# YuhuaXu/ImageMosaicing

Measured on AMD Instinct MI355X. Metric: image-pairs/sec (detect+match+H+warp), 4000x3000 UAV frames, higher is better.
Workload: dtype i16 fixed-point pyramid filtered in f32 (as the reference's OpenCV), f32 (RANSAC / warp coordinates), int8 MFMA with int32 accumulation (descriptor distances, exact), u8 (pixels); 1 GPU; C3: ONE 500-frame 4000x3000 UAV survey, pair window 2 (499 pairs), SIFT(2000,3,0.01,20) + exact BF match + 3x3 grid select + Ransac2D + MosaicImagesRefined warp; frames=500, pairs=499, frames_per_gpu=500, pairs_per_gpu=499

## Files before the change

imagemosaicing_amd/csrc/sift.hip:

```cpp
#include "common.h"
#include <memory>
#include "detmath.h"
#include <cmath>
#include <type_traits>

namespace {

constexpr int N_LAYERS = 3, N_LEVELS = 6, IMG_BORDER = 5, MAX_INTERP = 5, ORI_BINS = 36, MAX_OCT = 16;
constexpr int FIXPT_SCALE = 48;
constexpr float DOG_THRESHOLD_P1 = 21.0f;
constexpr float HIST_Q = 1024.0f;
constexpr int MAX_R = 16;
constexpr int SIFT_BATCH_MAX = MI355_SIFT_BATCH_MAX;
typedef int16_t lvl_t;

__host__ __device__ __forceinline__ int reflect101(int p, int n) {
    if (n == 1) return 0;
    while (p < 0 || p >= n) { if (p < 0) p = -p; else p = 2 * n - 2 - p; }
    return p;
}

typedef float v2f __attribute__((ext_vector_type(2)));
struct __attribute__((aligned(4))) uint2_a4 { unsigned x, y; };
typedef float v4f __attribute__((ext_vector_type(4)));
// ... 546 lines not shown
        for (int idx = lane; idx < nq; idx += 64) {
            const unsigned g = base + (unsigned)idx;
            if (g >= cap) { *overflow = 1; continue; }
            cand[(size_t)reg * cap + g] = s_rec[wave][idx];
        }
        wave_sync();
        nq = 0;
    };
    auto emit = [&](unsigned hit, int rc, auto in_loop) -> bool {
        constexpr bool IN_LOOP = decltype(in_loop)::value;
        const int nq0 = nq;
        while (__builtin_amdgcn_ballot_w64(hit != 0)) {
            const bool mine = hit != 0;
            const int bb = mine ? __builtin_ctz(hit) : 0;
            hit &= hit - 1;
            const unsigned long long m = __builtin_amdgcn_ballot_w64(mine);
            const int add = __builtin_popcountll(m);
            if (nq + add > XCAP) {
                if constexpr (IN_LOOP) { nq = nq0; return false; }
                else flush();
            }
            if (mine) {
                const int layer = bb / 4 + 1, c = xm + (bb & 3);
                s_rec[wave][nq + __builtin_popcountll(m & ((1ull << lane) - 1ull))] =
                    ((unsigned long long)octave << 48) | ((unsigned long long)layer << 40) | ((unsigned long long)rc << 20) | (unsigned long long)c;
            }
            nq += add;
        }
        return true;
    };
    XH win[3];
    XCen cen[3];
    XRow nxt[XD];
    {
        XRow q; XDog dq;
        load_row(y0 - 1, q); to_dog(q, dq); xrow_extremes(dq, win[0], cen[0]);
        load_row(y0, q); to_dog(q, dq); xrow_extremes(dq, win[1], cen[1]);
#pragma unroll
        for (int d = 0; d < XD; d++) load_row(y0 + 1 + d, nxt[d]);
    }
    int tb = 0, t_slow = -1;
    for (bool done = false; !done;) {
        for (;;) {
            if (tb >= lact) { done = true; break; }
            if (nq > XCAP / 2) break;
            auto step = [&](auto jc) -> bool {
                constexpr int j = decltype(jc)::value;
                const int tt = tb + j;
                if (tt >= lact) return false;
                const int rc = y0 + tt;
                XH& A = win[j % 3]; XH& B = win[(j + 1) % 3]; XH& Cc = win[(j + 2) % 3];
                { XDog dq; to_dog(nxt[j % XD], dq); xrow_extremes(dq, Cc, cen[(j + 2) % 3]); }
                load_row(rc + 1 + XD, nxt[j % XD]);
                const unsigned hit = xtest_rows(A, B, Cc, cen[(j + 1) % 3], xm, clo, chi, rc >= IMG_BORDER && rc < oc.h - IMG_BORDER);
                if (!emit(hit, rc, std::true_type{})) { t_slow = tt; return false; }
                return true;
            };
            if (!static_rows<0, 3 * XD>(step)) { done = true; break; }
            tb += 3 * XD;
        }
        flush();
    }
    if (t_slow >= 0) {
        for (int tt = t_slow; tt < lact; tt++) {
            const int rc = y0 + tt;
            XRow q; XDog A, B, Cc;
            load_row(rc - 1, q); to_dog(q, A);
            load_row(rc, q); to_dog(q, B);
            load_row(rc + 1, q); to_dog(q, Cc);
            emit(xtest_row(A, B, Cc, xm, clo, chi, rc >= IMG_BORDER && rc < oc.h - IMG_BORDER), rc, std::false_type{});
        }
        flush();
    }
}

__global__ __launch_bounds__(256) void refine_kernel(PyrDev P, const unsigned long long* cand_all, const unsigned* cand_counts, unsigned cand_cap, unsigned* cand_total,
                                                     float contrast_thr, float edge_thr, float sigma,
                                                     Refined* out, unsigned* out_count, unsigned out_cap, unsigned* out_resp, BatchStride bs,
                                                     const float* cube_all, unsigned cube_cap) {
    const size_t fr = blockIdx.z, foff = fr * bs.pyr;
    cube_all += fr * bs.cube;
    cand_all += fr * bs.cand; cand_counts += fr * CCNT_STRIDE; cand_total += fr * CNT_STRIDE;
    out += fr * bs.refined; out_count += fr * CNT_STRIDE; out_resp += fr * bs.refined;
    const unsigned reg = blockIdx.y;
    unsigned n = cand_counts[reg * REG_STRIDE];
    if (n > cand_cap) n = cand_cap;
    const unsigned long long* cand = cand_all + (size_t)reg * cand_cap;
    if (blockIdx.x == 0 && blockIdx.y == 0 && threadIdx.x < 64) {
        unsigned tot = cand_counts[threadIdx.x * REG_STRIDE];
        for (int off = 32; off > 0; off >>= 1) tot += __shfl_xor(tot, off);
        if (threadIdx.x == 0) cand_total[0] = tot;
    }
    for (unsigned i = blockIdx.x * blockDim.x + threadIdx.x; i < n; i += gridDim.x * blockDim.x) {
        const unsigned long long pk = cand[i];
        const int o = (int)((pk >> 48) & 0xff);
        int L = (int)((pk >> 40) & 0xff), R = (int)((pk >> 20) & 0xfffff), C = (int)(pk & 0xfffff);
        const unsigned start = ((unsigned)L << 28) | ((unsigned)R << 14) | (unsigned)C;
        const OctaveDev& oc = P.oc[o];
        auto dv = [&](int l, int r, int c) { return dogv(oc, foff, l, r, c); };
        FitOff f = {0.0f, 0.0f, 0.0f};
        int it = 0;
        bool alive = true, accepted = false;
        float contr = 0.0f;
        const bool from_cube = (pk >> 63) != 0;
        const bool can_gather = (oc.w & 1) == 0 && (foff & 1) == 0;
        float cv[27];
        auto gather = [&](int l, int r, int c) {
            const int a0 = (c - 1) & ~1, sh = ((c - 1) & 1) * 16;
            int v[4][9];
#pragma unroll
            for (int q = 0; q < 4; q++) {
                const lvl_t* lp = oc.lv[l - 1 + q] + foff;
#pragma unroll
                for (int dr = 0; dr < 3; dr++) {
                    const uint2_a4 wv = *reinterpret_cast<const uint2_a4*>(lp + (size_t)(r - 1 + dr) * oc.w + a0);
                    const unsigned long long ww = (((unsigned long long)wv.y << 32) | wv.x) >> sh;
                    v[q][dr * 3 + 0] = (int)(short)(ww & 0xffffu); v[q][dr * 3 + 1] = (int)(short)((ww >> 16) & 0xffffu); v[q][dr * 3 + 2] = (int)(short)((ww >> 32) & 0xffffu);
                }
            }
#pragma unroll
            for (int dl = 0; dl < 3; dl++)
#pragma unroll
                for (int e = 0; e < 9; e++) cv[dl * 9 + e] = (float)(v[dl + 1][e] - v[dl][e]);
        };
        if (from_cube || can_gather) {
            for (; it < MAX_INTERP; it++) {
                if (it == 0 && from_cube) {
                    const float* cb = cube_all + (size_t)reg * 32 * cube_cap + i;
#pragma unroll
                    for (int e = 0; e < 27; e++) cv[e] = cb[(size_t)e * cube_cap];
                } else if (can_gather) gather(L, R, C);
                else break;
                const int L0 = L, R0 = R, C0 = C;
                auto dvc = [&](int l, int r, int c) { return cv[(l - L0 + 1) * 9 + (r - R0 + 1) * 3 + (c - C0 + 1)]; };
                f = fit_step(dvc, L, R, C);
                const int stt = fit_state(f);
                if (stt == 1) { alive = false; break; }
                if (stt == 0) { accepted = fit_accept(dvc, L, R, C, f, contrast_thr, edge_thr, contr); alive = accepted; break; }
                C += (int)rintf(f.xc); R += (int)rintf(f.xr); L += (int)rintf(f.xi);
                if (L < 1 || L > N_LAYERS || C < IMG_BORDER || C >= oc.w - IMG_BORDER || R < IMG_BORDER || R >= oc.h - IMG_BORDER) { alive = false; break; }
            }
            if (!alive || (can_gather && !accepted)) continue;
        }
        if (!accepted) {
            for (; it < MAX_INTERP; it++) {
                f = fit_step(dv, L, R, C);
                const int stt = fit_state(f);
                if (stt == 0) break;
                if (stt == 1) { alive = false; break; }
                C += (int)rintf(f.xc); R += (int)rintf(f.xr); L += (int)rintf(f.xi);
                if (L < 1 || L > N_LAYERS || C < IMG_BORDER || C >= oc.w - IMG_BORDER || R < IMG_BORDER || R >= oc.h - IMG_BORDER) { alive = false; break; }
            }
            if (!alive || it >= MAX_INTERP) continue;
            if (!fit_accept(dv, L, R, C, f, contrast_thr, edge_thr, contr)) continue;
        }
        const size_t bit = ((size_t)R * oc.w + C) * 4 + (size_t)L;
        const unsigned mask = 1u << (bit & 31);
        if (!P.mins[o]) {
            const unsigned old = atomicOr(&P.claimed[o][fr * bs.claimed + (bit >> 5)], mask);
            if (old & mask) continue;
        }
        const unsigned long long act = __ballot(1);
        const int leader = __builtin_ctzll(act), lane_id = (int)(threadIdx.x & 63);
        unsigned slot = 0;
        if (lane_id == leader) slot = atomicAdd(out_count, (unsigned)__builtin_popcountll(act));
        slot = __shfl(slot, leader) + (unsigned)__builtin_popcountll(act & ((1ull << lane_id) - 1ull));
        if (slot < out_cap) {
            Refined rr;
            rr.o = o; rr.layer = L; rr.r = R; rr.c = C; rr.xi = f.xi; rr.xr = f.xr; rr.xc = f.xc; rr.contr = contr;
            rr.scl = sigma * det_exp2f(((float)L + f.xi) / (float)N_LAYERS);
            rr.start = start;
            out[slot] = rr;
            out_resp[slot] = __float_as_uint(fabsf(contr));
            if (P.mins[o]) atomicMin(&P.mins[o][fr * bs.mins + bit], start);
        } else if (!P.mins[o]) atomicAnd(&P.claimed[o][fr * bs.claimed + (bit >> 5)], ~mask);
    }
}

__device__ __forceinline__ void unclaim_body(const PyrDev& P, const Refined* ref, const unsigned* ref_count, unsigned ref_cap, const BatchStride& bs, size_t fr, unsigned first, unsigned step) {
    ref += fr * bs.refined; ref_count += fr * CNT_STRIDE;
    unsigned n = *ref_count;
    if (n > ref_cap) n = ref_cap;
    for (unsigned i = first; i < n; i += step) {
        const Refined rr = ref[i];
        const size_t bit = ((size_t)rr.r * P.oc[rr.o].w + rr.c) * 4 + (size_t)rr.layer;
        atomicAnd(&P.claimed[rr.o][fr * bs.claimed + (bit >> 5)], ~(1u << (bit & 31)));
    }
}

__global__ __launch_bounds__(256) void keepall_live_kernel(PyrDev P, const Refined* ref, const unsigned* ref_count, unsigned ref_cap, unsigned* ctrl, unsigned* list, BatchStride bs) {
    const size_t fr = blockIdx.y;
    ref += fr * bs.refined; ref_count += fr * CNT_STRIDE; ctrl += fr * CNT_STRIDE; list += fr * bs.refined;
    unsigned n = *ref_count;
    if (n > ref_cap) n = ref_cap;
    const int lane = threadIdx.x & 63;
    for (unsigned i0 = blockIdx.x * blockDim.x; i0 < n; i0 += gridDim.x * blockDim.x) {
        const unsigned i = i0 + threadIdx.x;
        bool take = false;
        if (i < n) {
            const Refined rr = ref[i];
            const size_t bit = ((size_t)rr.r * P.oc[rr.o].w + rr.c) * 4 + (size_t)rr.layer;
            take = P.mins[rr.o][fr * bs.mins + bit] == rr.start;
        }
        const unsigned long long m = __builtin_amdgcn_ballot_w64(take);
        if (m) {
            const int first = __builtin_ctzll(m);
            unsigned base = 0;
            if (lane == first) base = atomicAdd(&ctrl[2], (unsigned)__builtin_popcountll(m));
            base = __shfl(base, first);
            if (take) list[base + (unsigned)__builtin_popcountll(m & ((1ull << lane) - 1ull))] = i;
        }
    }
}
__global__ __launch_bounds__(256) void keepall_reset_kernel(PyrDev P, const Refined* ref, const unsigned* ref_count, unsigned ref_cap, BatchStride bs) {
    const size_t fr = blockIdx.y;
    ref += fr * bs.refined; ref_count += fr * CNT_STRIDE;
    unsigned n = *ref_count;
    if (n > ref_cap) n = ref_cap;
    for (unsigned i = blockIdx.x * blockDim.x + threadIdx.x; i < n; i += gridDim.x * blockDim.x) {
        const Refined rr = ref[i];
        P.mins[rr.o][fr * bs.mins + ((size_t)rr.r * P.oc[rr.o].w + rr.c) * 4 + (size_t)rr.layer] = 0xffffffffu;
    }
}

struct KpRec {
    unsigned resp_bits; int o, layer, r, c, bin;
    float ptx, pty, scl, angle, xi;
    unsigned start;
};

constexpr int UNCLAIM_WGS = 32;
__global__ __launch_bounds__(1024) void select_unclaim_kernel(PyrDev P, const Refined* ref, BatchStride bs,
                                                              const unsigned* resp , const unsigned* ref_count, unsigned ref_cap,
                                                              unsigned want, unsigned* ctrl , size_t resp_stride,
                                                              unsigned* list ) {
    if (blockIdx.x > 0) { unclaim_body(P, ref, ref_count, ref_cap, bs, blockIdx.y, (blockIdx.x - 1) * 1024 + threadIdx.x, (gridDim.x - 1) * 1024); return; }
    resp += (size_t)blockIdx.y * resp_stride; ref_count += (size_t)blockIdx.y * CNT_STRIDE; ctrl += (size_t)blockIdx.y * CNT_STRIDE;
    list += (size_t)blockIdx.y * resp_stride;
    __shared__ unsigned s_h[16][256];
    __shared__ unsigned s_sel[2], s_cnt;
    const int tid = threadIdx.x, wv = tid >> 6;
    unsigned n = *ref_count;
    if (n > ref_cap) n = ref_cap;
    if (n <= want) {
        if (tid == 0) { ctrl[0] = 0; ctrl[1] = 0; ctrl[2] = n; }
        for (unsigned i = tid; i < n; i += 1024) list[i] = i;
        return;
    }
    const unsigned nr = (n + 1023u) & ~1023u;
    unsigned above = 0, hi_sel = 0;
    for (int pass = 0; pass < 2; pass++) {
        for (int i = tid; i < 16 * 256; i += 1024) (&s_h[0][0])[i] = 0;
        __syncthreads();
        for (unsigned i0 = tid; i0 < nr; i0 += 8 * 1024) {
            unsigned vv[8];
#pragma unroll
            for (int u = 0; u < 8; u++) { const unsigned i = i0 + 1024u * u; vv[u] = i < n ? resp[i] : 0u; }
#pragma unroll
            for (int u = 0; u < 8; u++) {
                if (i0 + 1024u * u >= n) continue;
                const unsigned key = (vv[u] >> 15) & 0xffffu;
                if (pass == 0) atomicAdd(&s_h[wv][key >> 8], 1u);
                else if ((key >> 8) == hi_sel) atomicAdd(&s_h[wv][key & 255u], 1u);
            }
        }
        __syncthreads();
        if (tid < 256) { unsigned t = 0; for (int w = 0; w < 16; w++) t += s_h[w][tid]; s_h[0][tid] = t; }
        __syncthreads();
        if (tid == 0) {
            unsigned cum = above; int b = 255;
            for (; b >= 0; b--) { if (cum + s_h[0][b] >= want) break; cum += s_h[0][b]; }
            if (b < 0) b = 0;
            s_sel[0] = (unsigned)b; s_sel[1] = cum;
        }
        __syncthreads();
        if (pass == 0) { hi_sel = s_sel[0]; above = s_sel[1]; }
        else if (tid == 0) { ctrl[0] = ((hi_sel << 8) | s_sel[0]) << 15; ctrl[1] = 0; s_cnt = 0; }
        __syncthreads();
    }
    const unsigned T = ((hi_sel << 8) | s_sel[0]) << 15;
    const int lane = tid & 63;
    for (unsigned i0 = tid; i0 < nr; i0 += 8 * 1024) {
        unsigned vv[8];
#pragma unroll
        for (int u = 0; u < 8; u++) { const unsigned i = i0 + 1024u * u; vv[u] = i < n ? resp[i] : 0u; }
#pragma unroll
        for (int u = 0; u < 8; u++) {
            const unsigned i = i0 + 1024u * u;
            const bool take = i < n && vv[u] >= T;
            const unsigned long long m = __builtin_amdgcn_ballot_w64(take);
            if (m) {
                const int first = __builtin_ctzll(m);
                unsigned base = 0;
                if (lane == first) base = atomicAdd(&s_cnt, (unsigned)__builtin_popcountll(m));
                base = __shfl(base, first);
                if (take) list[base + (unsigned)__builtin_popcountll(m & ((1ull << lane) - 1ull))] = i;
            }
        }
    }
    __syncthreads();
    if (tid == 0) ctrl[2] = s_cnt;
}

constexpr int OCAP = 256;
__global__ __launch_bounds__(256) void orient_kernel(PyrDev P, const Refined* ref, const unsigned* ref_count, unsigned ref_cap,
                                                     KpRec* out, unsigned* out_resp, unsigned* out_count, unsigned out_cap,
                                                     const unsigned* ctrl, int pass, BatchStride bs, const unsigned* list) {
    const size_t fr = blockIdx.y, foff = fr * bs.pyr;
    ref += fr * bs.refined; ref_count += fr * CNT_STRIDE; out += fr * bs.kps; out_resp += fr * bs.kps; out_count += fr * CNT_STRIDE; ctrl += fr * CNT_STRIDE;
    list += fr * bs.refined;
    __shared__ unsigned long long s_hq[4][ORI_BINS];
    const unsigned Tbits = ctrl[0];
    if (pass == 1 && (ctrl[1] == 0 || Tbits == 0)) return;
    __shared__ float s_hist[4][ORI_BINS + 4];
    __shared__ KpRec s_out[OCAP];
    __shared__ unsigned s_on, s_obase;
    const int tid = threadIdx.x, lane = tid & 63, wv = tid >> 6;
    unsigned n = *ref_count;
    if (n > ref_cap) n = ref_cap;
    if (pass == 0) n = ctrl[2] < n ? ctrl[2] : n;
    if (tid == 0) s_on = 0;
    __syncthreads();
    for (unsigned base = blockIdx.x * 4; base < n; base += gridDim.x * 4) {
        unsigned k = base + wv;
        bool take = false;
        if (k < n) {
            if (pass == 0) { k = list[k]; take = true; }
            else take = __float_as_uint(fabsf(ref[k].contr)) < Tbits;
        }
        if (take) {
            const Refined rr = ref[k];
            const OctaveDev& oc = P.oc[rr.o];
            const lvl_t* img = oc.lv[rr.layer] + foff;
            const int radius = (int)rintf(4.5f * rr.scl);
            const float osig = 1.5f * rr.scl;
            const float expf_scale = -1.0f / (2.0f * osig * osig);
            const int side = 2 * radius + 1, S = side * side;
            if (lane < ORI_BINS) s_hq[wv][lane] = 0ull;
            __builtin_amdgcn_fence(__ATOMIC_ACQ_REL, "workgroup");
            __builtin_amdgcn_wave_barrier();
            const int per = (S + 63) / 64;
            int sc = lane * per, ic = sc / side, jc = sc - ic * side;
            for (int k0 = 0; k0 < per; k0 += 4) {
                float dxv[4], dyv[4]; int d2v[4]; bool okv[4];
#pragma unroll
                for (int u = 0; u < 4; u++) {
                    const int s = k0 + u < per ? sc : S;
                    const int i = ic - radius, j = jc - radius;
                    sc++; jc++;
                    if (jc == side) { jc = 0; ic++; }
                    const int y = rr.r + i, x = rr.c + j;
                    okv[u] = (s < S) && !(y <= 0 || y >= oc.h - 1 || x <= 0 || x >= oc.w - 1);
                    d2v[u] = i * i + j * j;
                    dxv[u] = 0.0f; dyv[u] = 0.0f;
                    if (okv[u]) {
                        dxv[u] = (float)((int)img[(size_t)y * oc.w + x + 1] - (int)img[(size_t)y * oc.w + x - 1]);
                        dyv[u] = (float)((int)img[(size_t)(y - 1) * oc.w + x] - (int)img[(size_t)(y + 1) * oc.w + x]);
                    }
                }
#pragma unroll
                for (int u = 0; u < 4; u++) {
                    if (!okv[u]) continue;
                    const float dx = dxv[u], dy = dyv[u];
                    const float wgt = det_expf((float)d2v[u] * expf_scale);
                    const float ang = det_atan2deg(dy, dx);
                    const float mag = sqrtf(dx * dx + dy * dy);
                    int b = (int)rintf(((float)ORI_BINS / 360.0f) * ang);
                    if (b >= ORI_BINS) b -= ORI_BINS;
                    if (b < 0) b += ORI_BINS;
                    const float t = wgt * mag;
                    atomicAdd(&s_hq[wv][b], (unsigned long long)(long long)(int)rintf(t * HIST_Q));
                }
            }
            __builtin_amdgcn_fence(__ATOMIC_ACQ_REL, "workgroup");
            __builtin_amdgcn_wave_barrier();
            if (lane < ORI_BINS) s_hist[wv][lane] = (float)(long long)s_hq[wv][lane] * (1.0f / HIST_Q);
            __builtin_amdgcn_fence(__ATOMIC_ACQ_REL, "workgroup");
            __builtin_amdgcn_wave_barrier();
            float hs = 0.0f;
            if (lane < ORI_BINS) {
                const float m2 = s_hist[wv][(lane + ORI_BINS - 2) % ORI_BINS], m1 = s_hist[wv][(lane + ORI_BINS - 1) % ORI_BINS];
                const float p1 = s_hist[wv][(lane + 1) % ORI_BINS], p2 = s_hist[wv][(lane + 2) % ORI_BINS];
                hs = ((m2 + p2) * (1.0f / 16.0f) + (m1 + p1) * (4.0f / 16.0f)) + s_hist[wv][lane] * (6.0f / 16.0f);
            }
            float omax = hs;
            for (int off = 32; off > 0; off >>= 1) { const float o2 = __shfl_xor(omax, off); omax = o2 > omax ? o2 : omax; }
            const float hl = __shfl(hs, lane > 0 ? lane - 1 : ORI_BINS - 1);
            const float hr = __shfl(hs, lane < ORI_BINS - 1 ? lane + 1 : 0);
            const float mag_thr = omax * 0.8f;
            if (lane < ORI_BINS && hs > hl && hs > hr && hs >= mag_thr) {
                float bf = (float)lane + (0.5f * (hl - hr)) / ((hl - 2.0f * hs) + hr);
                bf = bf < 0.0f ? (float)ORI_BINS + bf : (bf >= (float)ORI_BINS ? bf - (float)ORI_BINS : bf);
                KpRec kr;
                kr.resp_bits = __float_as_uint(fabsf(rr.contr));
                kr.o = rr.o; kr.layer = rr.layer; kr.r = rr.r; kr.c = rr.c; kr.bin = lane;
                kr.ptx = (float)rr.c + rr.xc; kr.pty = (float)rr.r + rr.xr; kr.scl = rr.scl; kr.xi = rr.xi; kr.start = rr.start;
                kr.angle = (360.0f / (float)ORI_BINS) * bf;
                const unsigned slot = atomicAdd(&s_on, 1u);
                if (slot < OCAP) s_out[slot] = kr;
            }
        }
        __syncthreads();
        const bool last = base + gridDim.x * 4 >= n;
        if (s_on > OCAP - 72 || last) {
            const unsigned cntl = s_on < OCAP ? s_on : OCAP;
            if (tid == 0 && cntl) s_obase = atomicAdd(out_count, cntl);
            __syncthreads();
            for (unsigned i = tid; i < cntl; i += 256) {
                const unsigned g = s_obase + i;
                if (g < out_cap) { out[g] = s_out[i]; out_resp[g] = s_out[i].resp_bits; }
            }
            __syncthreads();
            if (tid == 0) s_on = 0;
            __syncthreads();
        }
    }
}

constexpr int TOPK_CAP = 4096;

struct SelRec { float ptx, pty, scl, angle; int o, layer; };

__device__ __forceinline__ unsigned long long tie_key(const KpRec& k) {
    return ((unsigned long long)k.o << 52) | ((unsigned long long)k.layer << 48) | ((unsigned long long)k.r << 28) | ((unsigned long long)k.c << 8) | (unsigned long long)k.bin;
}

__global__ __launch_bounds__(1024) void topk_kernel(const KpRec* kps, const unsigned* resp, const unsigned* kp_count, unsigned kp_cap, int nfeatures,
                                                    FrameOuts outs, SelRec* out_sel, int* out_n, int* overflow, unsigned* ctrl, int pass, BatchStride bs) {
    const size_t fr = blockIdx.x;
    kps += fr * bs.kps; resp += fr * bs.kps; kp_count += fr * CNT_STRIDE; out_sel += fr * bs.sel; out_n += fr * CNT_STRIDE; overflow += fr * CNT_STRIDE; ctrl += fr * CNT_STRIDE;
    mi355_keypoint* out_kp = outs.kp[0];
#pragma unroll
    for (int q = 1; q < SIFT_BATCH_MAX; q++) if ((int)fr == q) out_kp = outs.kp[q];
    __shared__ unsigned s_hist[256];
    if (pass == 1 && (ctrl[1] == 0 || ctrl[0] == 0)) return;
    __shared__ unsigned s_misc[8];
    __shared__ unsigned long long s_k0[TOPK_CAP];
    __shared__ unsigned long long s_k1[TOPK_CAP];
    __shared__ unsigned s_idx[TOPK_CAP];
    const int tid = threadIdx.x, lane = tid & 63;
    unsigned N = *kp_count;
    if (N > kp_cap) { N = kp_cap; if (tid == 0) *overflow = 1; }
    const unsigned K = (unsigned)nfeatures;
    unsigned thresh = 0;
    if (N > K) {
        unsigned prefix = 0, want = K;
        const unsigned Nr = (N + 1023u) & ~1023u;
        for (int pass = 0; pass < 4; pass++) {
            const int shift = 24 - 8 * pass;
            for (int i = tid; i < 256; i += 1024) s_hist[i] = 0;
            __syncthreads();
            const unsigned himask = pass == 0 ? 0u : (0xffffffffu << (shift + 8));
            for (unsigned i0 = tid; i0 < Nr; i0 += 8 * 1024) {
                unsigned vv[8];
#pragma unroll
                for (int u = 0; u < 8; u++) { const unsigned i = i0 + 1024u * u; vv[u] = i < N ? resp[i] : 0u; }
#pragma unroll
                for (int u = 0; u < 8; u++) {
                    const unsigned i = i0 + 1024u * u;
                    if (i0 + 1024u * u - tid >= Nr) break;
                    const unsigned v = vv[u];
                    const bool valid = (i < N) && ((v & himask) == prefix);
                    const unsigned d = (v >> shift) & 255u;
                    unsigned long long peers = __ballot(valid);
#pragma unroll
                    for (int b = 0; b < 8; b++) {
                        const unsigned long long m = __ballot(valid && ((d >> b) & 1u));
                        peers &= ((d >> b) & 1u) ? m : ~m;
                    }
                    if (valid && (peers & ((1ull << lane) - 1ull)) == 0ull) atomicAdd(&s_hist[d], (unsigned)__popcll(peers));
                }
            }
            __syncthreads();
            if (tid == 0) {
                unsigned cum = 0; int b = 255;
                for (; b >= 0; b--) { if (cum + s_hist[b] >= want) break; cum += s_hist[b]; }
                if (b < 0) b = 0;
                s_misc[0] = (unsigned)b; s_misc[1] = want - cum;
            }
            __syncthreads();
            prefix |= s_misc[0] << shift; want = s_misc[1];
            __syncthreads();
        }
        thresh = prefix;
    }
    if (tid == 0) s_misc[2] = 0;
    for (int i = tid; i < TOPK_CAP; i += 1024) { s_k0[i] = ~0ull; s_k1[i] = ~0ull; s_idx[i] = 0xffffffffu; }
    __syncthreads();
    for (unsigned i0 = tid; i0 < N; i0 += 8 * 1024) {
        unsigned vv[8];
#pragma unroll
        for (int u = 0; u < 8; u++) { const unsigned i = i0 + 1024u * u; vv[u] = i < N ? resp[i] : 0u; }
#pragma unroll
        for (int u = 0; u < 8; u++) {
            const unsigned i = i0 + 1024u * u;
            if (i < N && vv[u] >= thresh) {
                const KpRec k = kps[i];
                const unsigned slot = atomicAdd(&s_misc[2], 1u);
                if (slot < TOPK_CAP) { s_k0[slot] = (unsigned long long)(~k.resp_bits); s_k1[slot] = tie_key(k); s_idx[slot] = i; }
            }
        }
    }
    __syncthreads();
    unsigned M = s_misc[2];
    if (M > TOPK_CAP) { M = TOPK_CAP; if (tid == 0) *overflow = 1; }
    if (N > K && M > (unsigned)SEL_STRIDE && tid == 0) *overflow = 1;
    int SN = 64;
    while ((unsigned)SN < M) SN <<= 1;
    for (int k = 2; k <= SN; k <<= 1) {
        for (int j = k >> 1; j > 0; j >>= 1) {
            for (int i = tid; i < SN; i += 1024) {
                const int ixj = i ^ j;
                if (ixj > i) {
                    const unsigned long long a0 = s_k0[i], a1 = s_k1[i], b0 = s_k0[ixj], b1 = s_k1[ixj];
                    const bool gt = (a0 > b0) || (a0 == b0 && a1 > b1);
                    const bool up = (i & k) == 0;
                    if (gt == up) {
                        s_k0[i] = b0; s_k1[i] = b1; s_k0[ixj] = a0; s_k1[ixj] = a1;
                        const unsigned t = s_idx[i]; s_idx[i] = s_idx[ixj]; s_idx[ixj] = t;
                    }
                }
            }
            __syncthreads();
        }
    }
    const unsigned keep = N > K ? (M < (unsigned)SEL_STRIDE ? M : (unsigned)SEL_STRIDE) : M;
    for (unsigned i = tid; i < keep; i += 1024) {
        const KpRec k = kps[s_idx[i]];
        const float s2 = (float)(1 << k.o);
        mi355_keypoint kp;
        kp.x = k.ptx * s2; kp.y = k.pty * s2; kp.size = (k.scl * s2) * 2.0f; kp.angle = k.angle;
        kp.response = __uint_as_float(k.resp_bits);
        kp.octave = (k.o & 255) | (k.layer << 8) | (((int)rintf((k.xi + 0.5f) * 255.0f)) << 16);
        kp.class_id = -1;
        out_kp[i] = kp;
        SelRec sr; sr.ptx = k.ptx; sr.pty = k.pty; sr.scl = k.scl; sr.angle = k.angle; sr.o = k.o; sr.layer = k.layer;
        out_sel[i] = sr;
    }
    if (tid == 0) {
        *out_n = (int)keep;
        if (pass == 0 && ctrl[0] != 0 && keep < K) ctrl[1] = 1;
    }
}

__global__ __launch_bounds__(256) void keepall_output_kernel(const KpRec* kps, const unsigned* kp_count, unsigned kp_cap, FrameOuts outs, SelRec* out_sel, int* out_n, int* overflow, BatchStride bs) {
    const size_t fr = blockIdx.y;
    kps += fr * bs.kps; kp_count += fr * CNT_STRIDE; out_sel += fr * bs.sel; out_n += fr * CNT_STRIDE; overflow += fr * CNT_STRIDE;
    mi355_keypoint* out_kp = outs.kp[0];
#pragma unroll
    for (int q = 1; q < SIFT_BATCH_MAX; q++) if ((int)fr == q) out_kp = outs.kp[q];
    unsigned N = *kp_count;
    if (N > kp_cap || N > (unsigned)KEEPALL_MAX) {
        if (blockIdx.x == 0 && threadIdx.x == 0) { *overflow = 1; *out_n = 0; }
        return;
    }
    if (blockIdx.x == 0 && threadIdx.x == 0) *out_n = (int)N;
    auto key_of = [](const KpRec& k) { return ((unsigned long long)k.o << 40) | ((unsigned long long)k.start << 6) | (unsigned long long)k.bin; };
    __shared__ unsigned long long s_key[1024];
    const unsigned i = blockIdx.x * 256 + threadIdx.x;
    if (blockIdx.x * 256 >= N) return;
    KpRec mine;
    unsigned long long mk = ~0ull;
    if (i < N) { mine = kps[i]; mk = key_of(mine); }
    unsigned rank = 0;
    for (unsigned t0 = 0; t0 < N; t0 += 1024) {
        __syncthreads();
        for (unsigned q = threadIdx.x; q < 1024; q += 256) s_key[q] = t0 + q < N ? key_of(kps[t0 + q]) : ~0ull;
        __syncthreads();
        const unsigned cntq = N - t0 < 1024 ? N - t0 : 1024;
        for (unsigned q = 0; q < cntq; q++) rank += s_key[q] < mk ? 1u : 0u;
    }
    if (i >= N) return;
    const KpRec& k = mine;
    const float s2 = (float)(1 << k.o);
    mi355_keypoint kp;
    kp.x = k.ptx * s2; kp.y = k.pty * s2; kp.size = (k.scl * s2) * 2.0f; kp.angle = k.angle;
    kp.response = __uint_as_float(k.resp_bits);
    kp.octave = (k.o & 255) | (k.layer << 8) | (((int)rintf((k.xi + 0.5f) * 255.0f)) << 16);
    kp.class_id = -1;
    out_kp[rank] = kp;
    SelRec sr; sr.ptx = k.ptx; sr.pty = k.pty; sr.scl = k.scl; sr.angle = k.angle; sr.o = k.o; sr.layer = k.layer;
    out_sel[rank] = sr;
}

__global__ __launch_bounds__(256) void describe_kernel(PyrDev P, const SelRec* sel, const int* n_sel, FrameOuts outs, BatchStride bs) {
    const size_t fr = blockIdx.y, foff = fr * bs.pyr;
    sel += fr * bs.sel; n_sel += fr * CNT_STRIDE;
    uint8_t* desc = outs.d8[0];
#pragma unroll
    for (int q = 1; q < SIFT_BATCH_MAX; q++) if ((int)fr == q) desc = outs.d8[q];
    constexpr int d = 4, n = 8, HB = (d + 2) * (d + 2) * (n + 2);
    __shared__ unsigned long long s_hq4[4][HB];
    __shared__ float s_dst4[4][128];
    const int lane = threadIdx.x & 63, wv = threadIdx.x >> 6;
    const int kidx = blockIdx.x * 4 + wv;
    if (kidx >= *n_sel) return;
    unsigned long long* s_hq = s_hq4[wv];
    float* s_dst = s_dst4[wv];
    auto wave_sync = [&]() { __builtin_amdgcn_fence(__ATOMIC_ACQ_REL, "workgroup"); __builtin_amdgcn_wave_barrier(); };
    const SelRec k = sel[kidx];
    const OctaveDev& oc = P.oc[k.o];
    const lvl_t* img = oc.lv[k.layer] + foff;
    const int rows = oc.h, cols = oc.w;
    for (int i = lane; i < HB; i += 64) s_hq[i] = 0ull;
    wave_sync();
    const int px = (int)rintf(k.ptx), py = (int)rintf(k.pty);
    float sin_t, cos_t;
    det_sincosdeg(k.angle, sin_t, cos_t);
    const float bins_per_deg = (float)n / 360.0f;
    const float exp_scale = -1.0f / ((float)(d * d) * 0.5f);
    const float hist_width = 3.0f * k.scl;
    const int radius = (int)rintf(hist_width * 1.4142135623730951f * (float)(d + 1) * 0.5f);
    cos_t = cos_t / hist_width; sin_t = sin_t / hist_width;
    const int side = 2 * radius + 1, S = side * side;
    __shared__ int s_q4[4][64 * 5];
    int* s_q = s_q4[wv];
    int qn = 0;
    auto heavy = [&](int packed) {
        const int i = (int)((unsigned)packed >> 16) - 32768, j = (int)((unsigned)packed & 0xffffu) - 32768;
        const float c_rot = (float)j * cos_t - (float)i * sin_t;
        const float r_rot = (float)j * sin_t + (float)i * cos_t;
        float rbin = r_rot + (float)(d / 2) - 0.5f;
        float cbin = c_rot + (float)(d / 2) - 0.5f;
        const int r = py + i, c = px + j;
        const float dx = (float)((int)img[(size_t)r * cols + c + 1] - (int)img[(size_t)r * cols + c - 1]);
        const float dy = (float)((int)img[(size_t)(r - 1) * cols + c] - (int)img[(size_t)(r + 1) * cols + c]);
        const float ori = det_atan2deg(dy, dx);
        const float mag = sqrtf(dx * dx + dy * dy) * det_expf((c_rot * c_rot + r_rot * r_rot) * exp_scale);
        float obin = (ori - k.angle) * bins_per_deg;
        const float r0f = floorf(rbin), c0f = floorf(cbin), o0f = floorf(obin);
        rbin -= r0f; cbin -= c0f; obin -= o0f;
        const int r0 = (int)r0f, c0 = (int)c0f;
        int o0 = (int)o0f;
        if (o0 < 0) o0 += n;
        if (o0 >= n) o0 -= n;
        const float v_r1 = mag * rbin, v_r0 = mag - v_r1;
        const float v_rc11 = v_r1 * cbin, v_rc10 = v_r1 - v_rc11;
        const float v_rc01 = v_r0 * cbin, v_rc00 = v_r0 - v_rc01;
        const float v_rco111 = v_rc11 * obin, v_rco110 = v_rc11 - v_rco111;
        const float v_rco101 = v_rc10 * obin, v_rco100 = v_rc10 - v_rco101;
        const float v_rco011 = v_rc01 * obin, v_rco010 = v_rc01 - v_rco011;
        const float v_rco001 = v_rc00 * obin, v_rco000 = v_rc00 - v_rco001;
        const int idx = ((r0 + 1) * (d + 2) + c0 + 1) * (n + 2) + o0;
#define FIXQ(v) ((unsigned long long)(long long)(int)rintf((v) * HIST_Q))
        atomicAdd(&s_hq[idx], FIXQ(v_rco000)); atomicAdd(&s_hq[idx + 1], FIXQ(v_rco001));
        atomicAdd(&s_hq[idx + (n + 2)], FIXQ(v_rco010)); atomicAdd(&s_hq[idx + (n + 3)], FIXQ(v_rco011));
        atomicAdd(&s_hq[idx + (d + 2) * (n + 2)], FIXQ(v_rco100)); atomicAdd(&s_hq[idx + (d + 2) * (n + 2) + 1], FIXQ(v_rco101));
        atomicAdd(&s_hq[idx + (d + 3) * (n + 2)], FIXQ(v_rco110)); atomicAdd(&s_hq[idx + (d + 3) * (n + 2) + 1], FIXQ(v_rco111));
#undef FIXQ
    };
    const int per = (S + 63) / 64;
    int sc = lane * per, ic = sc / side, jc = sc - ic * side;
    for (int k0 = 0; k0 < per; k0 += 4) {
#pragma unroll
        for (int u = 0; u < 4; u++) {
            const int kk = k0 + u;
            const int i = ic - radius, j = jc - radius;
            const float c_rot = (float)j * cos_t - (float)i * sin_t;
            const float r_rot = (float)j * sin_t + (float)i * cos_t;
            const float rbin = r_rot + (float)(d / 2) - 0.5f;
            const float cbin = c_rot + (float)(d / 2) - 0.5f;
            const int r = py + i, c = px + j;
            const bool ok = kk < per && sc < S && (rbin > -1.0f && rbin < (float)d && cbin > -1.0f && cbin < (float)d && r > 0 && r < rows - 1 && c > 0 && c < cols - 1);
            const unsigned long long m = __builtin_amdgcn_ballot_w64(ok);
            if (ok) s_q[qn + __builtin_popcountll(m & ((1ull << lane) - 1ull))] = (int)(((unsigned)(i + 32768) << 16) | (unsigned)(j + 32768));
            qn += __builtin_popcountll(m);
            sc++; jc++;
            if (jc == side) { jc = 0; ic++; }
        }
        wave_sync();
        while (qn >= 64) {
            qn -= 64;
            heavy(s_q[qn + lane]);
        }
        wave_sync();
    }
    if (lane < qn) heavy(s_q[lane]);
    wave_sync();
#pragma unroll
    for (int half = 0; half < 2; half++) {
        const int t = lane + 64 * half;
        const int cell = t >> 3, q = t & 7, i = cell >> 2, j = cell & 3;
        const int idx = ((i + 1) * (d + 2) + (j + 1)) * (n + 2);
        float v = (float)(long long)s_hq[idx + q] * (1.0f / HIST_Q);
        if (q < 2) v = v + (float)(long long)s_hq[idx + n + q] * (1.0f / HIST_Q);
        s_dst[t] = v;
    }
    wave_sync();
    float a = s_dst[lane], b = s_dst[lane + 64];
    auto seq_sum = [&](float va, float vb) {
        const float sa = va * va, sb = vb * vb;
        float acc = 0.0f;
#pragma unroll
        for (int q = 0; q < 64; q++) acc = acc + __int_as_float(__builtin_amdgcn_readlane(__float_as_int(sa), q));
#pragma unroll
        for (int q = 0; q < 64; q++) acc = acc + __int_as_float(__builtin_amdgcn_readlane(__float_as_int(sb), q));
        return acc;
    };
    const float thr = sqrtf(seq_sum(a, b)) * 0.2f;
    a = a < thr ? a : thr; b = b < thr ? b : thr;
    const float nn = sqrtf(seq_sum(a, b));
    const float fac = 512.0f / (nn > 1.1920929e-7f ? nn : 1.1920929e-7f);
    const float va = rintf(a * fac), vb = rintf(b * fac);
    desc[(size_t)kidx * 128 + lane] = (uint8_t)(va < 0.0f ? 0 : (va > 255.0f ? 255 : (int)va));
    desc[(size_t)kidx * 128 + lane + 64] = (uint8_t)(vb < 0.0f ? 0 : (vb > 255.0f ? 255 : (int)vb));
}

int gauss_kernel_host(double sigma, float* k) {
    const int ksize = ((int)lrint(sigma * 8.0 + 1.0)) | 1;
    const int r = ksize / 2;
    double sum = 0.0;
    const double scale2x = -0.5 / (sigma * sigma);
    for (int i = 0; i < ksize; i++) { const double x = (double)i - (double)(ksize - 1) * 0.5; k[i] = (float)std::exp(scale2x * x * x); sum += (double)k[i]; }
    sum = 1.0 / sum;
    for (int i = 0; i < ksize; i++) k[i] = (float)((double)k[i] * sum);
    return r;
}
// ... 477 lines not shown
```

Before: 3888 image-pairs/s.

## Make orientation kernel wave-independent and clip histogram window to image bounds

```diff
diff --git a/imagemosaicing_amd/csrc/sift.hip b/imagemosaicing_amd/csrc/sift.hip
--- a/imagemosaicing_amd/csrc/sift.hip
+++ b/imagemosaicing_amd/csrc/sift.hip
@@ -872,32 +872,32 @@
     if (tid == 0) ctrl[2] = s_cnt;
 }
 
-constexpr int OCAP = 256;
+constexpr int OCAP_W = 64;
 __global__ __launch_bounds__(256) void orient_kernel(PyrDev P, const Refined* ref, const unsigned* ref_count, unsigned ref_cap,
                                                      KpRec* out, unsigned* out_resp, unsigned* out_count, unsigned out_cap,
                                                      const unsigned* ctrl, int pass, BatchStride bs, const unsigned* list) {
     const size_t fr = blockIdx.y, foff = fr * bs.pyr;
     ref += fr * bs.refined; ref_count += fr * CNT_STRIDE; out += fr * bs.kps; out_resp += fr * bs.kps; out_count += fr * CNT_STRIDE; ctrl += fr * CNT_STRIDE;
     list += fr * bs.refined;
-    __shared__ unsigned long long s_hq[4][ORI_BINS];
+    __shared__ unsigned long long s_hq4[4][ORI_BINS];
     const unsigned Tbits = ctrl[0];
     if (pass == 1 && (ctrl[1] == 0 || Tbits == 0)) return;
-    __shared__ float s_hist[4][ORI_BINS + 4];
-    __shared__ KpRec s_out[OCAP];
-    __shared__ unsigned s_on, s_obase;
+    __shared__ float s_hist4[4][ORI_BINS + 4];
+    __shared__ KpRec s_out4[4][OCAP_W];
     const int tid = threadIdx.x, lane = tid & 63, wv = tid >> 6;
+    unsigned long long* s_hq = s_hq4[wv];
+    float* s_hist = s_hist4[wv];
+    KpRec* s_out = s_out4[wv];
+    auto wave_sync = [&]() { __builtin_amdgcn_fence(__ATOMIC_ACQ_REL, "workgroup"); __builtin_amdgcn_wave_barrier(); };
     unsigned n = *ref_count;
     if (n > ref_cap) n = ref_cap;
     if (pass == 0) n = ctrl[2] < n ? ctrl[2] : n;
-    if (tid == 0) s_on = 0;
-    __syncthreads();
-    for (unsigned base = blockIdx.x * 4; base < n; base += gridDim.x * 4) {
-        unsigned k = base + wv;
-        bool take = false;
-        if (k < n) {
-            if (pass == 0) { k = list[k]; take = true; }
-            else take = __float_as_uint(fabsf(ref[k].contr)) < Tbits;
-        }
+    unsigned on = 0;
+    for (unsigned kk = blockIdx.x * 4 + wv; kk < n; kk += gridDim.x * 4) {
+        unsigned k = kk;
+        bool take = true;
+        if (pass == 0) k = list[kk];
+        else take = __float_as_uint(fabsf(ref[kk].contr)) < Tbits;
         if (take) {
             const Refined rr = ref[k];
             const OctaveDev& oc = P.oc[rr.o];
@@ -905,28 +905,29 @@
             const int radius = (int)rintf(4.5f * rr.scl);
             const float osig = 1.5f * rr.scl;
             const float expf_scale = -1.0f / (2.0f * osig * osig);
-            const int side = 2 * radius + 1, S = side * side;
-            if (lane < ORI_BINS) s_hq[wv][lane] = 0ull;
-            __builtin_amdgcn_fence(__ATOMIC_ACQ_REL, "workgroup");
-            __builtin_amdgcn_wave_barrier();
+            const int ilo = max(-radius, 1 - rr.r), ihi = min(radius, oc.h - 2 - rr.r);
+            const int jlo = max(-radius, 1 - rr.c), jhi = min(radius, oc.w - 2 - rr.c);
+            const int W = jhi >= jlo ? jhi - jlo + 1 : 0, S = ihi >= ilo ? (ihi - ilo + 1) * W : 0;
+            if (lane < ORI_BINS) s_hq[lane] = 0ull;
+            wave_sync();
             const int per = (S + 63) / 64;
-            int sc = lane * per, ic = sc / side, jc = sc - ic * side;
+            int sc = lane * per, ic = W ? sc / W : 0, jc = sc - ic * W;
+            const int send = min(sc + per, S);
             for (int k0 = 0; k0 < per; k0 += 4) {
                 float dxv[4], dyv[4]; int d2v[4]; bool okv[4];
 #pragma unroll
                 for (int u = 0; u < 4; u++) {
-                    const int s = k0 + u < per ? sc : S;
-                    const int i = ic - radius, j = jc - radius;
-                    sc++; jc++;
-                    if (jc == side) { jc = 0; ic++; }
-                    const int y = rr.r + i, x = rr.c + j;
-                    okv[u] = (s < S) && !(y <= 0 || y >= oc.h - 1 || x <= 0 || x >= oc.w - 1);
+                    okv[u] = sc < send;
+                    const int i = ilo + ic, j = jlo + jc;
                     d2v[u] = i * i + j * j;
                     dxv[u] = 0.0f; dyv[u] = 0.0f;
                     if (okv[u]) {
+                        const int y = rr.r + i, x = rr.c + j;
                         dxv[u] = (float)((int)img[(size_t)y * oc.w + x + 1] - (int)img[(size_t)y * oc.w + x - 1]);
                         dyv[u] = (float)((int)img[(size_t)(y - 1) * oc.w + x] - (int)img[(size_t)(y + 1) * oc.w + x]);
                     }
+                    sc++; jc++;
+                    if (jc == W) { jc = 0; ic++; }
                 }
 #pragma unroll
                 for (int u = 0; u < 4; u++) {
@@ -939,26 +940,26 @@
                     if (b >= ORI_BINS) b -= ORI_BINS;
                     if (b < 0) b += ORI_BINS;
                     const float t = wgt * mag;
-                    atomicAdd(&s_hq[wv][b], (unsigned long long)(long long)(int)rintf(t * HIST_Q));
+                    atomicAdd(&s_hq[b], (unsigned long long)(long long)(int)rintf(t * HIST_Q));
                 }
             }
-            __builtin_amdgcn_fence(__ATOMIC_ACQ_REL, "workgroup");
-            __builtin_amdgcn_wave_barrier();
-            if (lane < ORI_BINS) s_hist[wv][lane] = (float)(long long)s_hq[wv][lane] * (1.0f / HIST_Q);
-            __builtin_amdgcn_fence(__ATOMIC_ACQ_REL, "workgroup");
-            __builtin_amdgcn_wave_barrier();
+            wave_sync();
+            if (lane < ORI_BINS) s_hist[lane] = (float)(long long)s_hq[lane] * (1.0f / HIST_Q);
+            wave_sync();
             float hs = 0.0f;
             if (lane < ORI_BINS) {
-                const float m2 = s_hist[wv][(lane + ORI_BINS - 2) % ORI_BINS], m1 = s_hist[wv][(lane + ORI_BINS - 1) % ORI_BINS];
-                const float p1 = s_hist[wv][(lane + 1) % ORI_BINS], p2 = s_hist[wv][(lane + 2) % ORI_BINS];
-                hs = ((m2 + p2) * (1.0f / 16.0f) + (m1 + p1) * (4.0f / 16.0f)) + s_hist[wv][lane] * (6.0f / 16.0f);
+                const float m2 = s_hist[(lane + ORI_BINS - 2) % ORI_BINS], m1 = s_hist[(lane + ORI_BINS - 1) % ORI_BINS];
+                const float p1 = s_hist[(lane + 1) % ORI_BINS], p2 = s_hist[(lane + 2) % ORI_BINS];
+                hs = ((m2 + p2) * (1.0f / 16.0f) + (m1 + p1) * (4.0f / 16.0f)) + s_hist[lane] * (6.0f / 16.0f);
             }
             float omax = hs;
             for (int off = 32; off > 0; off >>= 1) { const float o2 = __shfl_xor(omax, off); omax = o2 > omax ? o2 : omax; }
             const float hl = __shfl(hs, lane > 0 ? lane - 1 : ORI_BINS - 1);
             const float hr = __shfl(hs, lane < ORI_BINS - 1 ? lane + 1 : 0);
             const float mag_thr = omax * 0.8f;
-            if (lane < ORI_BINS && hs > hl && hs > hr && hs >= mag_thr) {
+            const bool peak = lane < ORI_BINS && hs > hl && hs > hr && hs >= mag_thr;
+            const unsigned long long pm = __builtin_amdgcn_ballot_w64(peak);
+            if (peak) {
                 float bf = (float)lane + (0.5f * (hl - hr)) / ((hl - 2.0f * hs) + hr);
                 bf = bf < 0.0f ? (float)ORI_BINS + bf : (bf >= (float)ORI_BINS ? bf - (float)ORI_BINS : bf);
                 KpRec kr;
@@ -966,23 +967,21 @@
                 kr.o = rr.o; kr.layer = rr.layer; kr.r = rr.r; kr.c = rr.c; kr.bin = lane;
                 kr.ptx = (float)rr.c + rr.xc; kr.pty = (float)rr.r + rr.xr; kr.scl = rr.scl; kr.xi = rr.xi; kr.start = rr.start;
                 kr.angle = (360.0f / (float)ORI_BINS) * bf;
-                const unsigned slot = atomicAdd(&s_on, 1u);
-                if (slot < OCAP) s_out[slot] = kr;
-            }
-        }
-        __syncthreads();
-        const bool last = base + gridDim.x * 4 >= n;
-        if (s_on > OCAP - 72 || last) {
-            const unsigned cntl = s_on < OCAP ? s_on : OCAP;
-            if (tid == 0 && cntl) s_obase = atomicAdd(out_count, cntl);
-            __syncthreads();
-            for (unsigned i = tid; i < cntl; i += 256) {
-                const unsigned g = s_obase + i;
-                if (g < out_cap) { out[g] = s_out[i]; out_resp[g] = s_out[i].resp_bits; }
-            }
-            __syncthreads();
-            if (tid == 0) s_on = 0;
-            __syncthreads();
+                s_out[on + (unsigned)__builtin_popcountll(pm & ((1ull << lane) - 1ull))] = kr;
+            }
+            on += (unsigned)__builtin_popcountll(pm);
+        }
+        if (on > (unsigned)(OCAP_W - 18) || (on && kk + gridDim.x * 4 >= n)) {
+            wave_sync();
+            unsigned obase = 0;
+            if (lane == 0) obase = atomicAdd(out_count, on);
+            obase = __shfl(obase, 0);
+            if ((unsigned)lane < on) {
+                const unsigned g = obase + lane;
+                if (g < out_cap) { out[g] = s_out[lane]; out_resp[g] = s_out[lane].resp_bits; }
+            }
+            wave_sync();
+            on = 0;
         }
     }
 }
```

Measured after the change: 3917 image-pairs/s (median of 6 runs). About the same (+0.7%).
